# ingonyama-zk/blaze

Hardware: AMD Instinct MI355X
Metric: BLS12-381 MSM/s at 2^26 (higher is better)
Workload: dtype u32 registers holding 28-bit limbs (381-bit Fq, Montgomery)

## Files before the change

blaze_amd/_lib.py:

```python
from __future__ import annotations

import ctypes as C
import os

_HERE = os.path.dirname(os.path.abspath(__file__))
LIB_PATH = os.environ.get("BLAZE_HIP_LIB") or os.path.join(_HERE, "lib", "libblaze_hip.so")


class DriverClientError(Exception):

    VARIANTS = {
        1: "WriteError",
        2: "ReadError",
        3: "HBICAPNotReady",
        4: "InvalidPrimitiveParam",
        5: "CsvError",
        6: "LoadFailed",
        7: "FileError",
        8: "Unknown",
    }

    def __init__(self, code: int, message: str):
        self.code = code
        self.variant = self.VARIANTS.get(code, "Unknown")
# ... 99 lines not shown
    "blz_poseidon_wait_result": (C.c_int, [C.c_void_p]),
    "blz_poseidon_num_pending_results": (C.c_int, [C.c_void_p, C.POINTER(C.c_uint32)]),
    "blz_poseidon_raw_results": (C.c_int, [C.c_void_p, C.c_uint32, _u8p, C.c_size_t]),
    "blz_poseidon_result": (C.c_int, [C.c_void_p, C.c_uint32, _u8p, C.c_size_t, C.POINTER(C.c_uint32)]),
    "blz_poseidon_tree_device": (C.c_int, [C.c_void_p, C.c_void_p, C.c_size_t]),
    "blz_poseidon_counters": (C.c_int, [C.c_void_p, C.POINTER(C.c_uint32)]),
    "blz_poseidon_info": (C.c_int, [C.c_void_p, C.POINTER(C.c_uint64)]),
    "blz_poseidon_set_round_plan": (C.c_int, [C.c_void_p, C.c_int]),
    "blz_poseidon_prepare_round_plan": (C.c_int, [C.c_void_p, C.POINTER(C.c_uint32)]),
    "blz_poseidon_last_kernel_ms": (C.c_int, [C.c_void_p, C.POINTER(C.c_float)]),
    "blz_poseidon_stream": (C.c_int, [C.c_void_p, C.POINTER(C.c_void_p), C.POINTER(C.c_int)]),
    "blz_poseidon_reset": (C.c_int, [C.c_void_p]),
    "blz_device_malloc": (C.c_int, [C.c_int, C.c_size_t, C.POINTER(C.c_void_p)]),
    "blz_device_free": (C.c_int, [C.c_int, C.c_void_p]),
    "blz_host_malloc": (C.c_int, [C.c_int, C.c_size_t, C.POINTER(C.c_void_p)]),
    "blz_host_free": (C.c_int, [C.c_void_p]),
    "blz_memcpy_h2d": (C.c_int, [C.c_int, C.c_void_p, _u8p, C.c_size_t]),
    "blz_memcpy_d2h": (C.c_int, [C.c_int, _u8p, C.c_void_p, C.c_size_t]),
}
EXPORTED_SYMBOLS = tuple(_SIGS)
_AUX_SIGS = {
    "blz_synth_scalars": (C.c_int, [C.c_int, C.c_int, C.c_void_p, C.c_uint64, C.c_uint64]),
    "blz_synth_scalars_at": (C.c_int, [C.c_int, C.c_int, C.c_void_p, C.c_uint64, C.c_uint64, C.c_uint64]),
    "blz_synth_points": (C.c_int, [C.c_int, C.c_int, C.c_void_p, C.c_uint64, C.c_int, C.c_uint64]),
    "blz_synth_field_elements": (C.c_int, [C.c_int, C.c_void_p, C.c_uint64, C.c_uint64]),
    "blz_calib_mad_rate": (C.c_int, [C.c_int, C.c_uint32, C.POINTER(C.c_double)]),
    "blz_test_msm_stall": (C.c_int, [C.c_void_p, C.c_uint32, C.POINTER(C.c_void_p)]),
    "blz_test_ntt_stall": (C.c_int, [C.c_void_p, C.c_uint32, C.POINTER(C.c_void_p)]),
    "blz_test_stall_release": (C.c_int, [C.c_void_p]),
    "blz_test_field_op": (C.c_int, [C.c_int, C.c_int, C.c_int, C.c_int, _u8p, _u8p, _u8p, C.c_size_t]),
    "blz_test_ec_op": (C.c_int, [C.c_int, C.c_int, C.c_int, _u8p, _u8p, _u8p, _u8p, _u8p, C.c_size_t]),
    "blz_test_msm_tail_plan": (C.c_int, [C.c_int, C.c_int, C.c_uint32, C.c_int, C.c_int, C.c_int, C.c_int, C.c_int, C.POINTER(C.c_uint32), C.POINTER(C.c_uint8),
                                         C.c_char_p, C.c_size_t]),
    "blz_test_poseidon_permute": (C.c_int, [C.c_int, C.c_int, _u8p, C.c_size_t, C.c_int, _u8p, _u8p, C.c_size_t]),
    "blz_test_poseidon_hash": (C.c_int, [C.c_int, C.c_int, _u8p, C.c_size_t, C.c_int, _u8p, _u8p, C.c_size_t]),
    "blz_test_poseidon_hash_plan": (C.c_int, [C.c_int, C.c_int, _u8p, C.c_size_t, C.c_int, _u8p, _u8p, C.c_size_t, C.POINTER(C.c_uint32)]),
    "blz_test_poseidon_tree_check": (C.c_int, [C.c_int, C.c_int, _u8p, C.c_size_t, C.c_int, C.c_uint32, C.c_void_p, C.c_void_p, C.POINTER(C.c_uint64)]),
}
AUX_EXPORTED_SYMBOLS = tuple(_AUX_SIGS)


def lib():
    global _lib
    if _lib is None:
        if not os.path.exists(LIB_PATH):
            raise RuntimeError(
                f"{LIB_PATH} is missing: build it with `make -C blaze_amd/csrc` "
                "(or __graft_entry__.build()); blaze_amd has no CPU fallback"
            )
        L = C.CDLL(LIB_PATH, mode=C.RTLD_GLOBAL)
        for name, (res, args) in _SIGS.items():
            fn = getattr(L, name)
            fn.restype = res
            fn.argtypes = args
        _lib = L
    return _lib


def aux():
    global _aux
    if _aux is None:
        lib()
        path = LIB_PATH[:-3] + "_aux.so"
        if not os.path.exists(path):
            raise RuntimeError(f"{path} is missing: build it with `make -C blaze_amd/csrc`")
        A = C.CDLL(path)
# ... 93 lines not shown
```

blaze_amd/csrc/msm.hip:

```cpp
#include "msm_engine.hpp"
#include <mutex>
#include "field.hip.hpp"
#include "msm_digits.hip.hpp"

namespace blz {

size_t fq_bytes(int curve) { return curve == BLZ_BN254 ? 32 : 48; }
size_t mont_point_bytes(int curve) { return curve == BLZ_BN254 ? 64 : 128; }

static MsmPlan search_plan(uint32_t npts, int sbits, int ebits, int force_c, int split_ns, int max_w) {
    MsmPlan best;
    double best_cost = 1e300;
    const double t_entry = 0.163, t_bucket = 0.62, t_empty = 0.03, t_hot = 0.01;
    const int need = sbits + 1;
    const double t_split = (double)split_ns;
    for (int cmin = 3; cmin <= 23; ++cmin) {
        if (force_c > 0 && cmin != force_c) continue;
        for (int W = 1; W <= max_w; ++W) {
            if ((uint64_t)npts * W > MSM_MAX_ENTRIES) break;
            const int lower = W - 1;
            for (int k = 0; k <= lower; ++k) {
                if (force_c > 0 && k != 0) break;
                if (k > 0 && cmin + 1 > 23) break;
                const int low_bits = lower * cmin + k;
// ... 592 lines not shown
}

int MsmEngine::sync_all() {
    BLZ_TRY(use_device(device));
    BLZ_TRY(sync_stream_bounded(stream, "reset: main stream"));
    BLZ_TRY(sync_stream_bounded(tail_stream, "reset: tail stream"));
    BLZ_TRY(sync_stream_bounded(aux_stream, "reset: exchange stream"));
    BLZ_TRY(sync_stream_bounded(sort_stream, "reset: sort stream"));
    for (auto& S : slots) { S.busy = false; S.open = false; S.task_inputs_event = nullptr; }
    return BLZ_OK;
}

int MsmEngine::points_to_mont(const void* d_raw, void* d_mont, uint32_t npts) {
    BLZ_TRY(use_device(device));
    return msm_ops_for(curve, repr)->points_to_mont(*this, d_raw, d_mont, npts);
}

int MsmEngine::points_to_mont_even(const void* d_raw, void* d_mont, uint32_t nq) {
    BLZ_TRY(use_device(device));
    return msm_ops_for(curve, repr)->points_to_mont_even(*this, d_raw, d_mont, nq);
}
int MsmEngine::check_precompute(const void* d_raw, uint64_t nelem, uint32_t* flag, hipStream_t st) {
    BLZ_TRY(use_device(device));
    return msm_ops_for(curve, 0)->check_precompute(*this, d_raw, nelem, flag, st);
}

int MsmEngine::build_table(const void* d_raw, void* d_table, uint32_t npts, int c, int W, int base_shift, void* scratch, uint32_t* flag,
                           hipStream_t st) {
    BLZ_TRY(use_device(device));
    return msm_ops_for(curve, repr)->build_table(*this, d_raw, d_table, npts, c, W, base_shift, scratch, flag, st);
}
size_t MsmEngine::table_scratch_bytes(int W) const { return msm_ops_for(curve, repr)->table_scratch_bytes(W); }

static bool sort_fits_beside(int av, int sv) {
    const int a = (av + 7) & ~7, s = (sv + 7) & ~7;
    int waves = 512 / a;
    if (waves > 4) waves = 4;
    if (waves < 1) waves = 1;
    return waves * a + s <= 512 - 32;
}

static const int kScalarFieldBits[3] = {253, 255, 254};

MsmPlan MsmEngine::plan_for(uint32_t npts, int sbits) const {
    const int ebits = sbits == 256 ? kScalarFieldBits[curve] : sbits;
    return make_plan(npts, sbits, ebits, plan_override("c", 0));
}

static MsmPlan range_plan(int curve, uint32_t npts, int bit_lo, int bit_hi) {
    const int vbits = bit_hi - bit_lo;
    int ebits = kScalarFieldBits[curve] - bit_lo;
    if (ebits > vbits) ebits = vbits;
    if (ebits < 1) ebits = 1;
    MsmPlan P = make_plan(npts, vbits, ebits, plan_override("c", 0));
    P.base_bit = bit_lo;
    return P;
}
MsmPlan MsmEngine::plan_for_range(uint32_t npts, int bit_lo, int bit_hi) const { return range_plan(curve, npts, bit_lo, bit_hi); }

int msm_task_plan(int curve, uint32_t npts, int sbits, int table_c, int bit_lo, int bit_hi, MsmPlan& P, bool* ranged_out) {
    if (curve < 0 || curve > 2) return fail(BLZ_ERR_INVALID_PARAM, "unknown curve %d", curve);
    const int ebits = sbits == 256 ? kScalarFieldBits[curve] : sbits;
    const bool ranged = bit_hi > bit_lo && !(bit_lo == 0 && bit_hi >= sbits);
    if (ranged && (sbits != 256 || (bit_lo & 31) || (bit_hi & 31) || bit_hi > 256))
        return fail(BLZ_ERR_INVALID_PARAM, "scalar range [%d, %d): 32-bit aligned ranges of 256-bit scalars", bit_lo, bit_hi);
    P = table_c > 0 ? make_table_plan(npts, table_c, ranged ? bit_hi - bit_lo + 1 : 257)
        : ranged    ? range_plan(curve, npts, bit_lo, bit_hi)
                    : make_plan(npts, sbits, ebits, plan_override("c", 0));
    if (P.c == 0) return fail(BLZ_ERR_INVALID_PARAM, "no window plan for npts=%u sbits=%d%s", npts, sbits, table_c > 0 ? " (window table)" : "");
    if (P.table && !msm_sort3_ok(P, sbits)) return fail(BLZ_ERR_INVALID_PARAM, "window-table task outside the sort's range (c=%d)", P.c);
    P.L = (uint32_t)plan_override("L", (int)P.L);
    if (P.L < 1) P.L = 1;
// ... 9 lines not shown
    const uint32_t per = (uint32_t)(((2ull * P.npts + halves - 1) / halves + 15) & ~(uint64_t)15);
    if (want > 1) want = (int)(((uint64_t)P.npts + per - 1) / per);
    *per_out = want > 1 ? per : P.npts;
    return want;
}

int MsmEngine::begin(uint32_t npts, int sbits, int* slot_out, int table_c, int bit_lo, int bit_hi, int nslices, bool phased) {
    BLZ_TRY(use_device(device));
    const MsmCurveOps* ops = msm_ops_for(curve, repr);
    hipStream_t st = stream;
    if (npts == 0) return fail(BLZ_ERR_INVALID_PARAM, "begin: empty task");
    int slot = (cur + 1) % MSM_QUEUE_DEPTH;
    if (slots[slot].busy) slot = (slot + 1) % MSM_QUEUE_DEPTH;
    if (slots[slot].busy) return fail(BLZ_ERR_INVALID_PARAM, "task queue full (%d tasks in flight)", MSM_QUEUE_DEPTH);
    MsmSlot& S = slots[slot];
    MsmPlan P;
    bool ranged = false;
    BLZ_TRY(msm_task_plan(curve, npts, sbits, table_c, bit_lo, bit_hi, P, &ranged));
    const uint64_t G = P.G;
    uint32_t per = npts;
    nslices = msm_task_pieces(P, nslices, phased, &per);
    BLZ_TRY(plan_tail(P, ops->tail, nslices > 1, S.tail));
    BLZ_LOG(2, "msm plan: npts=%u sbits=%d c=%d W=%d Bw=%u G=%llu L=%u pieces=%d tail: %s", npts, sbits, P.c, P.W, P.Bw,
            (unsigned long long)G, P.L, nslices, describe(S.tail).c_str());
    const uint64_t max_entries = (uint64_t)per * P.W;
    const uint64_t max_units = G + max_entries / P.L + 1;
    if (max_units >= (1ull << 32)) return fail(BLZ_ERR_INVALID_PARAM, "unit bound %llu exceeds 32 bits", (unsigned long long)max_units);

    const int hide_env = env_int("BLAZE_SORT_HIDE", 1);
    const MsmSlot& O = slots[(slot + 1) % MSM_QUEUE_DEPTH];
    bool s3 = P.table || (hide_env != 0 && nslices == 1 && msm_sort3_ok(P, sbits));
    bool fits = true;
    auto sort_fits = [&](bool table) {
        const int av = ops->accumulate_vgprs(), sv = msm_sort3_max_vgprs(table);
        return !(av > 0 && sv > 0 && !sort_fits_beside(av, sv));
    };
    if (s3 && hide_env == 1 && !P.table) {
        if (recent_hot[0] || recent_hot[1]) s3 = false;
    }
    if (s3 && hide_env == 1) {
        fits = sort_fits(P.table);
        if (!fits && !P.table) s3 = false;
    }
    bool hide = s3 && O.busy && hide_env != 0 && fits;
    const bool pingpong = nslices > 1 && hide_env != 0 && !O.busy && !P.table && msm_sort3_ok(P, sbits) && !(recent_hot[0] || recent_hot[1]) &&
                          sort_fits(false);
    if (pingpong) { s3 = true; hide = true; }

    cur = slot;
    if (slot_out) *slot_out = slot;
    last_plan = S.plan = P;
    S.npts = npts;
    S.sbits = sbits;
    S.ranged = ranged;
    S.bit_lo = bit_lo;
    S.bit_hi = bit_hi;
    S.repr = repr;
    S.slices = nslices;
    S.pts_per_slice = per;
    S.max_units = max_units;
    S.use_s3 = s3 && (hide || hide_env == 2 || P.table);
    S.sort_hidden = hide;
    S.pingpong = pingpong;
    S.acc_pp_recorded[0] = S.acc_pp_recorded[1] = false;
    S.phased = phased;
    S.task_inputs_event = inputs_event;
    S.accum_timed = false;
    BLZ_HIP(hipEventRecord(S.ev[0], st), BLZ_ERR_UNKNOWN);
// ... 230 lines not shown
```

blaze_amd/csrc/msm_engine.hpp:

```cpp
#pragma once
#include "common.hpp"

namespace blz {

constexpr int MSM_MAX_W = 96;
constexpr uint64_t MSM_MAX_ENTRIES = (1ull << 32) - (1ull << 26);
struct MsmPlan {
    uint32_t npts = 0;
    int sbits = 256;
    int c = 0;
    int W = 0;
    uint8_t width[MSM_MAX_W] = {};
    uint32_t boff[MSM_MAX_W + 1] = {};
    uint32_t Bw = 0;
    int Wv = 0;
    uint64_t G = 0;
    uint32_t L = 0;
    bool table = false;
    int ebits = 0;
    int base_bit = 0;
    double cost = 0;
};
MsmPlan make_plan(uint32_t npts, int sbits, int ebits, int force_c);
int table_window_bits(uint32_t npts, int need_bits = 257);
// ... 94 lines not shown
    bool last_sort_hidden = false;
    bool recent_hot[2] = {false, false};
    uint32_t sort_slices = 1, sort_nc = 0;
    int sort_cl = 0;
    void* sort_inter_fine = nullptr;

    int init(int device_id, int curve_id, int precompute_factor);
    bool destroy();
    uint32_t* slot_result(int s) { return result.as<uint32_t>() + (size_t)s * 64; }
    bool can_accept() const;
    MsmPlan plan_for(uint32_t npts, int sbits) const;
    int points_to_mont(const void* d_raw, void* d_mont, uint32_t npts);
    int points_to_mont_even(const void* d_raw, void* d_mont, uint32_t nq);
    int check_precompute(const void* d_raw, uint64_t nelem, uint32_t* flag, hipStream_t st);
    int build_table(const void* d_raw, void* d_table, uint32_t npts, int c, int W, int base_shift, void* scratch, uint32_t* flag,
                    hipStream_t st);
    size_t table_scratch_bytes(int W) const;
    int run(const void* d_points_mont, const void* d_scalars, uint32_t npts, int sbits, int* slot, int table_c = 0, int bit_lo = 0,
            int bit_hi = 0);
    MsmPlan plan_for_range(uint32_t npts, int bit_lo, int bit_hi) const;
    int finish(int slot, uint8_t* out);
    int combine_partials(const uint8_t* partials, size_t count, uint8_t* out, bool on_device);
    int sync_all();
};

int msm_points_from_mont(int format_id, const void* d_mont, void* d_raw, uint64_t npts, hipStream_t st);
int msm_points_all_canonical(int format_id, const void* d_raw, uint64_t npts, uint32_t* flag, hipStream_t st);
int copy_words_to_pinned(void* host_pinned, const void* d_src, uint32_t dwords, hipStream_t st);
size_t fq_bytes(int curve);
size_t mont_point_bytes(int curve);
int msm_sort_lds(MsmEngine& E, const void* d_scalars, uint32_t npts, int sbits);
bool msm_sort3_ok(const MsmPlan& P, int sbits);
int msm_sort3_max_vgprs(bool table);
int msm_sort3(MsmEngine& E, const void* d_scalars, uint32_t npts, int sbits);
int msm_sort_lds_scatter(MsmEngine& E);
bool msm_sort_tiny_ok(const MsmPlan& P, uint32_t npts, int sbits);
int msm_sort_tiny(MsmEngine& E, const void* d_scalars, uint32_t npts, int sbits, uint32_t max_units);
int launch_fill_units(MsmEngine& E, uint32_t units);

struct MsmCurveOps {
    int (*points_to_mont)(MsmEngine&, const void* d_raw, void* d_mont, uint32_t npts);
    int (*emit_infinity)(MsmEngine&);
    int (*run_accumulate)(MsmEngine&, MsmSlot&, const void* d_pts, uint32_t max_units, int slice);
    int (*merge_buckets)(MsmEngine&);
    int (*run_reduce)(MsmEngine&, MsmSlot&, const void* sums, const void* unit_off);
    TailTraits tail;
    int (*accumulate_vgprs)();
    int (*build_table)(MsmEngine&, const void* d_raw, void* d_table, uint32_t npts, int c, int W, int base_shift, void* scratch,
                       uint32_t* flag, hipStream_t st);
    size_t (*table_scratch_bytes)(int W);
    int (*combine)(MsmEngine&, const uint8_t* partials, size_t count, uint8_t* out, bool on_device);
    int (*points_to_mont_even)(MsmEngine&, const void* d_raw, void* d_mont, uint32_t nq);
    int (*check_precompute)(MsmEngine&, const void* d_raw, uint64_t nelem, uint32_t* flag, hipStream_t st);
    int (*points_from_mont)(const void* d_mont, void* d_raw, uint64_t npts, hipStream_t st);
    int (*points_all_canonical)(const void* d_raw, uint64_t npts, uint32_t* flag, hipStream_t st);
};
const MsmCurveOps& msm_ops_bls377();
const MsmCurveOps& msm_ops_bls381();
const MsmCurveOps& msm_ops_bn254();
const MsmCurveOps& msm_ops_bn254_w32();
const MsmCurveOps* msm_ops_for(int curve, int repr = 0);

}
```

blaze_amd/csrc/msm_impl.hip.hpp:

```cpp
#pragma once
#include "msm_engine.hpp"
#include "ec.hip.hpp"
#include "ec_rr.hip.hpp"
#include "ec_quad.hip.hpp"
#include "ec_row.hip.hpp"
#include <type_traits>

namespace blz {

template <class F>
constexpr int MONT_STRIDE = 2 * F::N > 16 ? 32 : 2 * F::N;

template <class F>
constexpr bool rr_point_packed() {
    if constexpr (USE_RR<F>) return 2 * F::RR::NL > MONT_STRIDE<F>;
    else return false;
}

template <class F>
BLZ_DEV void store_mont_point(uint32_t* __restrict__ mont, size_t p, Fp<F>& x, Fp<F>& y) {
    if constexpr (USE_RR<F>) {
        using Q = typename F::RR;
        Frr<Q, 1, 2> xr, yr;
        rr_to_mont_from_words<Q>(xr, x.v);
// ... 299 lines not shown
    if constexpr (USE_RR<F>) {
        XYZZRR<typename F::RR> r;
        ptrr_from_xyzz32<F>(r, a);
        ptrr_store(partial, idx, r);
    } else {
        uint32_t* q = partial + idx * 4 * F::N;
        fp_store(q, a.x); fp_store(q + F::N, a.y); fp_store(q + 2 * F::N, a.zz); fp_store(q + 3 * F::N, a.zzz);
    }
}

template <class F>
BLZ_DEV void load_affine(Affine<F>& a, const uint32_t* pts, uint32_t idx) {
    const uint32_t* q = pts + (size_t)idx * MONT_STRIDE<F>;
    fp_load(a.x, q);
    fp_load(a.y, q + F::N);
}
template <class F>
BLZ_DEV void load_xyzz(XYZZ<F>& a, const uint32_t* base, size_t idx) {
    const uint32_t* q = base + idx * 4 * F::N;
    fp_load(a.x, q);
    fp_load(a.y, q + F::N);
    fp_load(a.zz, q + 2 * F::N);
    fp_load(a.zzz, q + 3 * F::N);
}
template <class F>
BLZ_DEV void store_xyzz(uint32_t* base, size_t idx, const XYZZ<F>& a) {
    uint32_t* q = base + idx * 4 * F::N;
    fp_store(q, a.x);
    fp_store(q + F::N, a.y);
    fp_store(q + 2 * F::N, a.zz);
    fp_store(q + 3 * F::N, a.zzz);
}

#ifndef BLZ_ACC_RR_WAVES
#define BLZ_ACC_RR_WAVES 2
#endif
#ifndef BLZ_ACC_W32_WAVES
#define BLZ_ACC_W32_WAVES 2
#endif
#ifndef BLZ_ACC_VGPR_CAP
#define BLZ_ACC_VGPR_CAP 100
#endif
#ifdef BLZ_GATHER_MASK
#define BLZ_PT_IDX(e) ((e) & 0x7fffffffu & (uint32_t)(BLZ_GATHER_MASK))
#else
#define BLZ_PT_IDX(e) ((e) & 0x7fffffffu)
#endif
template <class F, bool CONT>
BLZ_DEV void accumulate_body(const uint32_t* __restrict__ pts, const uint32_t* __restrict__ entries,
                             const uint32_t* __restrict__ off, const uint32_t* __restrict__ unit_off,
                             const uint32_t* __restrict__ unit_bucket, const uint32_t* __restrict__ unit_order,
                             const uint32_t* __restrict__ stats, uint32_t L, uint32_t* __restrict__ partial,
                             uint32_t* __restrict__ sums, bool first) {
    uint32_t t = blockIdx.x * 128u + threadIdx.x;
    if (t >= stats[0]) return;
    const uint32_t u = unit_order[t];
    uint32_t g = unit_bucket[u];
    const uint32_t u0 = unit_off[g];
    uint32_t k = u - u0;
    uint32_t start = off[g] + k * L;
    uint32_t end = off[g + 1];
    if (end - start > L) end = start + L;
    uint32_t* dst = partial;
    size_t didx = u;
    bool resume = false;
    if constexpr (CONT) {
        if (unit_off[g + 1] - u0 == 1) {
            dst = sums;
            didx = g;
            resume = !first;
        }
    }
    if constexpr (USE_RR<F>) {
        using Q = typename F::RR;
        XYZZRR<Q> acc;
        ptrr_set_inf(acc);
        if constexpr (CONT) {
            if (resume) ptrr_load(acc, sums, g);
        }
        uint32_t e = entries[start];
#if BLZ_ACC_RR_WAVES == 2
        uint32_t en = start + 1 < end ? entries[start + 1] : 0u;
        AffineRR<Q> nxt;
        load_affine_rr<F>(nxt, pts, BLZ_PT_IDX(e));
        uint32_t j = start;
#ifndef BLZ_ACC_NO_AADD
        if ((!CONT || first) && end - start >= 2) {
            const AffineRR<Q> p0 = nxt;
            const bool neg0 = (e & 0x80000000u) != 0;
            const uint32_t e1 = en;
            AffineRR<Q> p1;
            load_affine_rr<F>(p1, pts, BLZ_PT_IDX(e1));
            if (start + 2 < end) {
                e = entries[start + 2];
                load_affine_rr<F>(nxt, pts, BLZ_PT_IDX(e));
                en = start + 3 < end ? entries[start + 3] : 0u;
            }
            ptrr_aadd<Q, 1>(acc, p0, neg0, p1, (e1 & 0x80000000u) != 0);
            j = start + 2;
        }
#endif
        for (; j < end; ++j) {
            const AffineRR<Q> cur = nxt;
            const bool neg = (e & 0x80000000u) != 0;
            if (j + 1 < end) {
                e = en;
                load_affine_rr<F>(nxt, pts, BLZ_PT_IDX(e));
                if (j + 2 < end) en = entries[j + 2];
            }
            ptrr_madd<Q, 1>(acc, cur, neg);
        }
// ... 892 lines not shown
    hipLaunchKernelGGL(k_points_all_canonical<F>, dim3((unsigned)((npts + 255) / 256)), dim3(256), 0, st, (const uint32_t*)d_raw, npts, flag);
    BLZ_HIP(hipGetLastError(), BLZ_ERR_UNKNOWN);
    return BLZ_OK;
}

constexpr uint32_t CHECK_BLOCKS = 256 * 4 * 3;
template <class F>
int points_to_mont_even_t(MsmEngine& E, const void* d_raw, void* d_mont, uint32_t nq) {
    if (nq == 0) return BLZ_OK;
    hipLaunchKernelGGL(k_points_to_mont_even<F>, dim3((nq + 255) / 256), dim3(256), 0, E.stream, (const uint32_t*)d_raw, (uint32_t*)d_mont, nq);
    BLZ_HIP(hipGetLastError(), BLZ_ERR_UNKNOWN);
    return BLZ_OK;
}
template <class F>
int check_precompute_t(MsmEngine& E, const void* d_raw, uint64_t nelem, uint32_t* flag, hipStream_t st) {
    (void)E;
    if (nelem == 0) return BLZ_OK;
    const uint64_t want = (nelem * 7u + 63u) / 64u;
    const uint32_t blocks = (uint32_t)(want < CHECK_BLOCKS ? want : CHECK_BLOCKS);
    hipLaunchKernelGGL(k_check_precompute<F>, dim3(blocks), dim3(64), 0, st, (const uint32_t*)d_raw, nelem, flag);
    BLZ_HIP(hipGetLastError(), BLZ_ERR_UNKNOWN);
    return BLZ_OK;
}

template <class F>
int accumulate_vgprs_t() {
    hipFuncAttributes a;
    if (hipFuncGetAttributes(&a, (const void*)k_accumulate<F>) != hipSuccess) {
        (void)hipGetLastError();
        return 0;
    }
    return a.numRegs;
}

template <class F>
MsmCurveOps make_ops() {
    MsmCurveOps o;
    o.points_to_mont = &points_to_mont_t<F>;
    o.emit_infinity = &emit_infinity_t<F>;
    o.run_accumulate = &run_accumulate_t<F>;
    o.merge_buckets = &merge_buckets_t<F>;
    o.run_reduce = &run_reduce_t<F>;
    o.tail = TailTraits{HAS_RR<F>, HAS_ROW<F>, partial_dwords<F>()};
    o.accumulate_vgprs = &accumulate_vgprs_t<F>;
    o.build_table = &build_table_t<F>;
    o.table_scratch_bytes = &table_scratch_bytes_t<F>;
    o.combine = &combine_t<F>;
    o.points_to_mont_even = &points_to_mont_even_t<F>;
    o.check_precompute = &check_precompute_t<F>;
    o.points_from_mont = &points_from_mont_t<F>;
    o.points_all_canonical = &points_all_canonical_t<F>;
    return o;
}

}
```

blaze_amd/csrc/msm_sort3.hip:

```cpp
#include "msm_engine.hpp"
#include "msm_digits.hip.hpp"

namespace blz {

constexpr int S3_THREADS = 256;
constexpr int S3_SH1 = 14;
constexpr int S3_SH2 = 7;
constexpr int S3_T = 12;
constexpr int S3_PB = S3_THREADS * S3_T;
constexpr uint32_t S3_SLICE2 = 4096;
constexpr int S3_T2 = S3_SLICE2 / S3_THREADS;
constexpr int S3_T3 = 28;
constexpr uint32_t S3_R3 = S3_THREADS * S3_T3;
constexpr uint32_t S3_MAXNB1 = 2048;
constexpr uint32_t S3_CNT_PTS = 16384;
constexpr uint32_t S3T_IMG = 12288;

struct S3Geom {
    int W, prio;
    uint32_t NB1;
    uint8_t width[MSM_MAX_W];
    uint16_t bitoff[MSM_MAX_W];
    uint16_t binoff1[MSM_MAX_W + 1];
    static constexpr bool TABLE = false;
    static constexpr uint32_t HIST1 = S3_MAXNB1;
    using Win = int;
    __device__ int cw(int w) const { return width[w]; }
    __device__ uint32_t first_bin(int w) const { return binoff1[w]; }
    __device__ static constexpr uint32_t shift1() { return S3_SH1; }
    static constexpr uint32_t bits3() { return S3_SH2; }
    __device__ static uint32_t index1(uint32_t p, uint32_t, uint32_t) { return p; }
    __device__ static uint32_t rem1(uint32_t rem) { return rem; }
    struct L2 {
        int prio;
        using Lo = uint8_t;
        static constexpr uint32_t TAB2 = 128;
        static constexpr uint32_t KY_D = 8, KY_R = 16;
        static constexpr uint32_t LO_MASK = 127u;
        __device__ static constexpr uint32_t shift2() { return S3_SH2; }
        __device__ static constexpr uint32_t bits2() { return S3_SH1 - S3_SH2; }
        __device__ static uint32_t low2(uint32_t r, uint32_t) { return r & 127u; }
// ... 567 lines not shown
    S3TGeom g;
    g.W = P.W;
    g.c = P.c;
    g.prio = exp_knob("BLAZE_SORT_PRIO", 3);
    g.sh1 = (uint32_t)(P.c - 1 - 8);
    g.NB1 = (uint32_t)(P.G >> g.sh1);
    const double per_bucket = (double)npts * P.W / (double)P.G;
    int b3 = 4;
    while (b3 < 10 && (double)(2u << b3) * per_bucket <= 6144.0) ++b3;
    if ((uint32_t)b3 > g.sh1) b3 = (int)g.sh1;
    int b2 = (int)g.sh1 - b3;
    if (b2 > 8) { b2 = 8; b3 = (int)g.sh1 - 8; }
    g.b2 = (uint32_t)b2;
    g.b3 = (uint32_t)b3;
    g.xs = g.sh1 > 16 ? g.sh1 - 16 : 0;
    return g;
}

bool msm_sort3_ok(const MsmPlan& P, int sbits) {
    if (P.table) {
        if (sbits != 256 || P.sbits < 1 || P.sbits > 256 || P.c < 16 || P.c > 26 || P.W * P.c < P.sbits + 1) return false;
        if ((uint64_t)P.npts * P.W >= (1ull << 30)) return false;
        const S3TGeom g = s3t_geometry(P, P.npts);
        return g.NB1 <= 256 && g.b2 <= 8 && g.b3 >= 1 && g.b3 <= 10 && g.xs <= 1 && g.b3 > g.xs;
    }
    if ((sbits != 256 && sbits != 64 && sbits != 32) || P.W < 1) return false;
    for (int w = 0; w < P.W; ++w)
        if (P.width[w] < S3_SH1 + 1 || P.width[w] > 23) return false;
    if ((P.G >> S3_SH1) > S3_MAXNB1 || (P.G & ((1u << S3_SH1) - 1u))) return false;
    if ((P.G >> S3_SH2) > 2048u * 256u) return false;
    return true;
}

int msm_sort3_max_vgprs(bool table) {
    using L2 = S3Geom::L2;
    static const void* const plain_ks[] = {(const void*)k3_l1_count<S3Geom, 8>, (const void*)k3_l1_scatter<S3Geom, 8>,
                                           (const void*)k3_l1_count<S3Geom, 1>, (const void*)k3_l1_scatter<S3Geom, 1>,
                                           (const void*)k3_l1_count<S3Geom, 2>, (const void*)k3_l1_scatter<S3Geom, 2>,
                                           (const void*)k3_l2_count<L2>, (const void*)k3_l2_scatter<L2>, (const void*)k3_l3};
    static const void* const table_ks[] = {(const void*)k3_l1_count<S3TGeom, 8>, (const void*)k3_l1_scatter<S3TGeom, 8>,
                                           (const void*)k3_l2_count<S3TGeom>, (const void*)k3_l2_scatter<S3TGeom>,
                                           (const void*)k3t_l3<true>, (const void*)k3t_l3<false>};
    static int cached[2] = {-1, -1};
    int& c = cached[table ? 1 : 0];
    if (c >= 0) return c;
    const void* const* ks = table ? table_ks : plain_ks;
    const size_t n = table ? sizeof(table_ks) / sizeof(*table_ks) : sizeof(plain_ks) / sizeof(*plain_ks);
    int mx = 0;
    for (size_t i = 0; i < n; ++i) {
        hipFuncAttributes a;
        if (hipFuncGetAttributes(&a, ks[i]) != hipSuccess) {
            (void)hipGetLastError();
            return c = 0;
        }
        if (a.numRegs > mx) mx = a.numRegs;
    }
    return c = mx;
}

template <class Geom, int NW>
static int s3_level1(hipStream_t st, const uint32_t* sc, uint32_t npts, const Geom& g, uint32_t* cnt1, uint32_t* off1, uint32_t* cur1,
                     uint32_t* i1_idx, uint16_t* i1_rem) {
    const dim3 blk(S3_THREADS);
    const size_t lds1 = (size_t)((NW + 2) * S3_PB + 3 * 256) * 4;
    hipLaunchKernelGGL((k3_l1_count<Geom, NW>), dim3((npts + S3_CNT_PTS - 1) / S3_CNT_PTS), blk, 0, st, sc, npts, g, cnt1);
    hipLaunchKernelGGL(k3_scan_small, dim3(1), blk, 0, st, cnt1, g.NB1, off1, cur1, g.prio);
    BLZ_TRY(ensure_dynamic_lds((const void*)k3_l1_scatter<Geom, NW>, (int)lds1));
    hipLaunchKernelGGL((k3_l1_scatter<Geom, NW>), dim3((npts + S3_PB - 1) / S3_PB), blk, lds1, st, sc, npts, g, cur1, i1_idx, i1_rem);
    return BLZ_OK;
}

template <class Geom>
static int s3_enqueue(MsmEngine& E, const Geom& g, const void* d_scalars, uint32_t npts, int sbits) {
    using L2 = typename Geom::L2;
    using Lo = typename L2::Lo;
    const MsmPlan& P = E.last_plan;
    hipStream_t st = E.sort_st;
    MsmEngine::SortBufs& B = E.sb();
    const uint32_t NB1 = g.NB1, NB2 = (uint32_t)(P.G >> g.bits3());
    const uint64_t max_entries = (uint64_t)npts * P.W;
    const uint32_t max_items = (uint32_t)(max_entries / S3_SLICE2) + NB1 + 1;
    const uint32_t nsb = (NB2 + 2047u) / 2048u;
    if (Geom::TABLE && nsb > 256) return fail(BLZ_ERR_UNKNOWN, "window-table sort: %u final-level bins exceed the scan's range", NB2);
    const size_t tab_dw = (size_t)3 * (NB1 + 2) + (size_t)3 * (NB2 + 2) + 260 + 4 + 2 * ((size_t)max_items + 2);
    BLZ_TRY(E.sort3_tabs.reserve(tab_dw * 4));
    uint32_t* cnt1 = E.sort3_tabs.as<uint32_t>();
    uint32_t* off1 = cnt1 + NB1 + 2;
    uint32_t* cur1 = off1 + NB1 + 2;
    uint32_t* cnt2 = cur1 + NB1 + 2;
    uint32_t* off2 = cnt2 + NB2 + 2;
    uint32_t* cur2 = off2 + NB2 + 2;
    uint32_t* bsum = cur2 + NB2 + 2;
    uint32_t* nitems = bsum + 260;
    uint2* map = reinterpret_cast<uint2*>(nitems + 4);
    BLZ_TRY(E.inter.reserve(max_entries * 6 + 64));
    BLZ_TRY(E.inter2.reserve(max_entries * (4 + sizeof(Lo)) + 64));
    uint32_t* i1_idx = E.inter.as<uint32_t>();
// ... 43 lines not shown
```

blaze_amd/csrc/testhooks.hip:

```cpp
#include "common.hpp"
#include "ec_rr.hip.hpp"
#include "ec_row.hip.hpp"
#include "poseidon_engine.hpp"
#include "msm_engine.hpp"

namespace blz {

template <class P>
__global__ __launch_bounds__(64) void k_test_field(int op, const uint32_t* a, const uint32_t* b, uint32_t* out, uint32_t n) {
    uint32_t i = blockIdx.x * 64u + threadIdx.x;
    if (i >= n) return;
    Fp<P> x, y, r;
    fp_load(x, a + (size_t)i * P::N);
    fp_load(y, b + (size_t)i * P::N);
    fp_to_mont(x, x);
    fp_to_mont(y, y);
    switch (op) {
        case 0: fp_mul(r, x, y); break;
        case 1: fp_add(r, x, y); break;
        case 2: fp_sub(r, x, y); break;
        case 3: fp_inv(r, x); break;
        case 5:
        case 6:
            if constexpr (P::LAZY) {
// ... 553 lines not shown
                                 const void* d_records, uint64_t out[2]) {
    if (!words || !d_input || !d_records || !out) return fail(BLZ_ERR_INVALID_PARAM, "null argument");
    if (tree_height < 1 || tree_height > 11) return fail(BLZ_ERR_INVALID_PARAM, "tree height out of range");
    BLZ_TRY(blz_poseidon_check_words(field, tree_mode, words, len, nullptr));
    BLZ_TRY(use_device(device_id));
    switch (field) {
        case BLZ_BLS377: return test_pos_tree_check_t<Fr_BLS377>(words, len, tree_mode, tree_height, d_input, d_records, out);
        case BLZ_BLS381: return test_pos_tree_check_t<Fr_BLS381>(words, len, tree_mode, tree_height, d_input, d_records, out);
        case BLZ_BN254: return test_pos_tree_check_t<Fr_BN254>(words, len, tree_mode, tree_height, d_input, d_records, out);
    }
    return fail(BLZ_ERR_INVALID_PARAM, "unknown field %d", field);
}

int blz_test_msm_tail_plan(int curve, int repr, uint32_t npts, int sbits, int pieces, int table_c, int bit_lo, int bit_hi, uint32_t plan_out[8],
                           uint8_t* widths, char* text, size_t cap) {
    if (!plan_out || !text || cap == 0) return fail(BLZ_ERR_INVALID_PARAM, "null argument");
    const MsmCurveOps* ops = msm_ops_for(curve, repr);
    if (!ops || npts == 0) return fail(BLZ_ERR_INVALID_PARAM, "unknown curve %d or empty task", curve);
    MsmPlan P;
    BLZ_TRY(msm_task_plan(curve, npts, sbits, table_c, bit_lo, bit_hi, P, nullptr));
    uint32_t per = 0;
    pieces = msm_task_pieces(P, pieces, false, &per);
    TailPlan T;
    BLZ_TRY(plan_tail(P, ops->tail, pieces > 1, T));
    const uint32_t out[8] = {(uint32_t)P.c, (uint32_t)P.W, (uint32_t)P.G, P.L, P.Bw, (uint32_t)P.Wv, (uint32_t)P.ebits, P.table ? 1u : 0u};
    memcpy(plan_out, out, sizeof(out));
    if (widths) memcpy(widths, P.width, (size_t)P.W);
    const std::string line = describe(T);
    if (line.size() >= cap) return fail(BLZ_ERR_INVALID_PARAM, "text buffer of %zu bytes for a line of %zu", cap, line.size());
    memcpy(text, line.c_str(), line.size() + 1);
    return BLZ_OK;
}

}
```

include/blaze_hip_aux.h:

```cpp
#ifndef BLAZE_HIP_AUX_H
#define BLAZE_HIP_AUX_H

#include "blaze_hip.h"

#ifdef __cplusplus
extern "C" {
#endif


int blz_synth_scalars(int device_id, int curve, void* d_out, uint64_t n, uint64_t seed);
int blz_synth_scalars_at(int device_id, int curve, void* d_out, uint64_t n, uint64_t seed, uint64_t start);
int blz_synth_points(int device_id, int curve, void* d_out, uint64_t n, int pf, uint64_t start);
int blz_synth_field_elements(int device_id, void* d_out, uint64_t n, uint64_t seed);

int blz_calib_mad_rate(int device_id, uint32_t target_ms, double out[4]);

int blz_test_msm_stall(blz_msm* h, uint32_t max_ms, void** token);
int blz_test_ntt_stall(blz_ntt* h, uint32_t max_ms, void** token);
int blz_test_stall_release(void* token);

int blz_test_field_op(int device_id, int curve, int field, int op, const uint8_t* a, const uint8_t* b,
                      uint8_t* out, size_t n);
int blz_test_ec_op(int device_id, int curve, int op, const uint8_t* p, const uint8_t* q,
                   const uint8_t* inf_flags, uint8_t* out, uint8_t* out_inf, size_t n);

int blz_test_msm_tail_plan(int curve, int repr, uint32_t npts, int sbits, int pieces, int table_c, int bit_lo, int bit_hi, uint32_t plan_out[8],
                           uint8_t* widths, char* text, size_t cap);

int blz_test_poseidon_permute(int device_id, int field, const uint8_t* words, size_t len, int t, const uint8_t* states_in,
                              uint8_t* states_out, size_t n);
int blz_test_poseidon_hash(int device_id, int field, const uint8_t* words, size_t len, int t, const uint8_t* inputs, uint8_t* digests,
                           size_t n);
int blz_test_poseidon_hash_plan(int device_id, int field, const uint8_t* words, size_t len, int t, const uint8_t* inputs, uint8_t* digests,
                                size_t n, uint32_t* state);
int blz_test_poseidon_tree_check(int device_id, int field, const uint8_t* words, size_t len, int tree_mode, uint32_t tree_height,
                                 const void* d_input, const void* d_records, uint64_t out[2]);

#ifdef __cplusplus
}
#endif
#endif
```

Before: 8.520.

## Gather bucket-accumulate points into LDS via async global_load_lds lines

In the RR accumulate kernel, each wave now brings point rows into LDS with global_load_lds. Lanes cooperatively fetch 128-byte point lines, using ds_swizzle to broadcast addresses, and the next point's load is double-buffered ahead of the madd. This is meant to replace scattered per-lane global point loads with coalesced line loads overlapped with arithmetic. The sort-hiding fit check now also counts LDS usage of the accumulate and sort3 kernels, and the sort3 per-thread tile drops from 12 to 8 so it fits beside the new LDS image. The costs are more LDS pressure, wave-uniform loop control where shorter buckets idle, and a hand-encoded gfx9 waitcnt.

Result: faster. 8.643 (median of 6 runs) (+1.4%).

```diff
diff --git a/blaze_amd/_lib.py b/blaze_amd/_lib.py
--- a/blaze_amd/_lib.py
+++ b/blaze_amd/_lib.py
@@ -155,6 +155,7 @@
     "blz_test_ec_op": (C.c_int, [C.c_int, C.c_int, C.c_int, _u8p, _u8p, _u8p, _u8p, _u8p, C.c_size_t]),
     "blz_test_msm_tail_plan": (C.c_int, [C.c_int, C.c_int, C.c_uint32, C.c_int, C.c_int, C.c_int, C.c_int, C.c_int, C.POINTER(C.c_uint32), C.POINTER(C.c_uint8),
                                          C.c_char_p, C.c_size_t]),
+    "blz_test_sort_fits_beside": (C.c_int, [C.c_int, C.c_int, C.c_int, C.c_int]),
     "blz_test_poseidon_permute": (C.c_int, [C.c_int, C.c_int, _u8p, C.c_size_t, C.c_int, _u8p, _u8p, C.c_size_t]),
     "blz_test_poseidon_hash": (C.c_int, [C.c_int, C.c_int, _u8p, C.c_size_t, C.c_int, _u8p, _u8p, C.c_size_t]),
     "blz_test_poseidon_hash_plan": (C.c_int, [C.c_int, C.c_int, _u8p, C.c_size_t, C.c_int, _u8p, _u8p, C.c_size_t, C.POINTER(C.c_uint32)]),
diff --git a/blaze_amd/csrc/msm.hip b/blaze_amd/csrc/msm.hip
--- a/blaze_amd/csrc/msm.hip
+++ b/blaze_amd/csrc/msm.hip
@@ -648,12 +648,16 @@
 }
 size_t MsmEngine::table_scratch_bytes(int W) const { return msm_ops_for(curve, repr)->table_scratch_bytes(W); }
 
-static bool sort_fits_beside(int av, int sv) {
+bool msm_sort_fits_beside(int av, int sv, int al, int sl) {
+    if (av <= 0 || sv <= 0) return true;
     const int a = (av + 7) & ~7, s = (sv + 7) & ~7;
     int waves = 512 / a;
     if (waves > 4) waves = 4;
     if (waves < 1) waves = 1;
-    return waves * a + s <= 512 - 32;
+    if (waves * a + s > 512 - 32) return false;
+    if (al <= 0 || sl <= 0) return true;
+    const int ak = (al + 1023) >> 10, sk = (sl + 1023) >> 10;
+    return 2 * waves * ak + sk <= 160;
 }
 
 static const int kScalarFieldBits[3] = {253, 255, 254};
@@ -729,8 +733,7 @@
     bool s3 = P.table || (hide_env != 0 && nslices == 1 && msm_sort3_ok(P, sbits));
     bool fits = true;
     auto sort_fits = [&](bool table) {
-        const int av = ops->accumulate_vgprs(), sv = msm_sort3_max_vgprs(table);
-        return !(av > 0 && sv > 0 && !sort_fits_beside(av, sv));
+        return msm_sort_fits_beside(ops->accumulate_vgprs(), msm_sort3_max_vgprs(table), ops->accumulate_lds(), msm_sort3_max_lds(table));
     };
     if (s3 && hide_env == 1 && !P.table) {
         if (recent_hot[0] || recent_hot[1]) s3 = false;
diff --git a/blaze_amd/csrc/msm_engine.hpp b/blaze_amd/csrc/msm_engine.hpp
--- a/blaze_amd/csrc/msm_engine.hpp
+++ b/blaze_amd/csrc/msm_engine.hpp
@@ -150,6 +150,8 @@
 int msm_sort_lds(MsmEngine& E, const void* d_scalars, uint32_t npts, int sbits);
 bool msm_sort3_ok(const MsmPlan& P, int sbits);
 int msm_sort3_max_vgprs(bool table);
+int msm_sort3_max_lds(bool table);
+bool msm_sort_fits_beside(int av, int sv, int al, int sl);
 int msm_sort3(MsmEngine& E, const void* d_scalars, uint32_t npts, int sbits);
 int msm_sort_lds_scatter(MsmEngine& E);
 bool msm_sort_tiny_ok(const MsmPlan& P, uint32_t npts, int sbits);
@@ -164,6 +166,7 @@
     int (*run_reduce)(MsmEngine&, MsmSlot&, const void* sums, const void* unit_off);
     TailTraits tail;
     int (*accumulate_vgprs)();
+    int (*accumulate_lds)();
     int (*build_table)(MsmEngine&, const void* d_raw, void* d_table, uint32_t npts, int c, int W, int base_shift, void* scratch,
                        uint32_t* flag, hipStream_t st);
     size_t (*table_scratch_bytes)(int W);
diff --git a/blaze_amd/csrc/msm_impl.hip.hpp b/blaze_amd/csrc/msm_impl.hip.hpp
--- a/blaze_amd/csrc/msm_impl.hip.hpp
+++ b/blaze_amd/csrc/msm_impl.hip.hpp
@@ -355,6 +355,52 @@
     fp_store(q + 3 * F::N, a.zzz);
 }
 
+template <class F>
+constexpr bool acc_gather_lines() {
+    if constexpr (USE_RR<F>) return !rr_point_packed<F>() && MONT_STRIDE<F> == 32 && F::RR::NL == 14;
+    else return false;
+}
+constexpr int ACC_IMG_PIECES = 512;
+template <int K>
+BLZ_DEV void acc_lines_issue_one(uint32_t lds, uint32_t lo, uint32_t hi, uint32_t piece) {
+    constexpr int pattern = (K << 5) | 0x18;
+    const uint32_t olo = (uint32_t)__builtin_amdgcn_ds_swizzle((int)lo, pattern);
+    const uint32_t ohi = (uint32_t)__builtin_amdgcn_ds_swizzle((int)hi, pattern);
+    const uint64_t src = (((uint64_t)ohi << 32) | olo) + piece;
+    __builtin_amdgcn_global_load_lds((const __attribute__((address_space(1))) void*)src,
+                                     (__attribute__((address_space(3))) void*)(uintptr_t)(lds + K * 1024), 16, 0, 0);
+}
+BLZ_DEV void acc_lines_issue(uint32_t lds, const uint32_t* pts, uint32_t idx) {
+    const uint64_t line = (uint64_t)(uintptr_t)pts + (uint64_t)idx * 128u;
+    const uint32_t lo = (uint32_t)line, hi = (uint32_t)(line >> 32), piece = (threadIdx.x & 7u) * 16u;
+    acc_lines_issue_one<0>(lds, lo, hi, piece); acc_lines_issue_one<1>(lds, lo, hi, piece);
+    acc_lines_issue_one<2>(lds, lo, hi, piece); acc_lines_issue_one<3>(lds, lo, hi, piece);
+    acc_lines_issue_one<4>(lds, lo, hi, piece); acc_lines_issue_one<5>(lds, lo, hi, piece);
+    acc_lines_issue_one<6>(lds, lo, hi, piece); acc_lines_issue_one<7>(lds, lo, hi, piece);
+}
+BLZ_DEV uint32_t acc_image_base(const uint4* img) {
+    return (uint32_t)__builtin_amdgcn_readfirstlane((int)(uint32_t)(uintptr_t)(const __attribute__((address_space(3))) void*)img);
+}
+template <class Q>
+BLZ_DEV void acc_lines_read(AffineRR<Q>& a, const uint4* img) {
+    const uint32_t lane = threadIdx.x & 63u;
+    const uint4* q4 = img + (lane & 7u) * 64 + (lane >> 3) * 8;
+    uint32_t w[2 * Q::NL];
+#if defined(__HIP_DEVICE_COMPILE__) && !defined(__GFX9__)
+#error "acc_lines_read: the s_waitcnt immediate is written in the gfx9 encoding"
+#endif
+    __builtin_amdgcn_s_waitcnt(0x0F70);
+    asm volatile("" ::: "memory");
+#pragma unroll
+    for (int i = 0; i < 2 * Q::NL / 4; ++i) {
+        uint4 v = q4[i];
+        w[4 * i] = v.x; w[4 * i + 1] = v.y; w[4 * i + 2] = v.z; w[4 * i + 3] = v.w;
+    }
+    asm volatile("s_waitcnt lgkmcnt(0)" ::: "memory");
+#pragma unroll
+    for (int i = 0; i < Q::NL; ++i) { a.x.v[i] = w[i]; a.y.v[i] = w[Q::NL + i]; }
+}
+
 #ifndef BLZ_ACC_RR_WAVES
 #define BLZ_ACC_RR_WAVES 2
 #endif
@@ -376,22 +422,33 @@
                              const uint32_t* __restrict__ stats, uint32_t L, uint32_t* __restrict__ partial,
                              uint32_t* __restrict__ sums, bool first) {
     uint32_t t = blockIdx.x * 128u + threadIdx.x;
-    if (t >= stats[0]) return;
-    const uint32_t u = unit_order[t];
-    uint32_t g = unit_bucket[u];
-    const uint32_t u0 = unit_off[g];
-    uint32_t k = u - u0;
-    uint32_t start = off[g] + k * L;
-    uint32_t end = off[g + 1];
-    if (end - start > L) end = start + L;
+#if BLZ_ACC_RR_WAVES == 2
+    constexpr bool LINES = acc_gather_lines<F>();
+#else
+    constexpr bool LINES = false;
+#endif
+    const uint32_t nunits = stats[0];
+    if ((LINES ? t & ~63u : t) >= nunits) return;
+    const bool live = t < nunits;
+    uint32_t g = 0, start = 0, end = 0;
     uint32_t* dst = partial;
-    size_t didx = u;
+    size_t didx = 0;
     bool resume = false;
-    if constexpr (CONT) {
-        if (unit_off[g + 1] - u0 == 1) {
-            dst = sums;
-            didx = g;
-            resume = !first;
+    if (live) {
+        const uint32_t u = unit_order[t];
+        g = unit_bucket[u];
+        const uint32_t u0 = unit_off[g];
+        const uint32_t k = u - u0;
+        start = off[g] + k * L;
+        end = off[g + 1];
+        if (end - start > L) end = start + L;
+        didx = u;
+        if constexpr (CONT) {
+            if (unit_off[g + 1] - u0 == 1) {
+                dst = sums;
+                didx = g;
+                resume = !first;
+            }
         }
     }
     if constexpr (USE_RR<F>) {
@@ -400,6 +457,50 @@
         ptrr_set_inf(acc);
         if constexpr (CONT) {
             if (resume) ptrr_load(acc, sums, g);
+        }
+        if constexpr (LINES) {
+            __shared__ uint4 images[2 * ACC_IMG_PIECES];
+            const uint4* img = images + (threadIdx.x >> 6) * ACC_IMG_PIECES;
+            const uint32_t lds = acc_image_base(img);
+            uint32_t j = start;
+            uint32_t e = j < end ? entries[j] : 0u;
+            uint32_t en = j + 1 < end ? entries[j + 1] : 0u;
+            acc_lines_issue(lds, pts, BLZ_PT_IDX(e));
+            if (live && start == end) ptrr_store(dst, didx, acc);
+#ifndef BLZ_ACC_NO_AADD
+            const bool aadd = (!CONT || first) && end - start >= 2;
+            if (__any(aadd)) {
+                AffineRR<Q> p0, p1;
+                acc_lines_read(p0, img);
+                const bool neg0 = (e & 0x80000000u) != 0;
+                const uint32_t e1 = aadd ? en : e;
+                acc_lines_issue(lds, pts, BLZ_PT_IDX(e1));
+                if (aadd) {
+                    j = start + 2;
+                    e = j < end ? entries[j] : 0u;
+                    en = j + 1 < end ? entries[j + 1] : 0u;
+                }
+                acc_lines_read(p1, img);
+                if (__any(j < end)) acc_lines_issue(lds, pts, BLZ_PT_IDX(e));
+                if (aadd) {
+                    ptrr_aadd<Q, 1>(acc, p0, neg0, p1, (e1 & 0x80000000u) != 0);
+                    if (j == end) ptrr_store(dst, didx, acc);
+                }
+            }
+#endif
+            while (__any(j < end)) {
+                AffineRR<Q> cur;
+                acc_lines_read(cur, img);
+                const bool neg = (e & 0x80000000u) != 0;
+                const bool more = j + 1 < end;
+                e = more ? en : 0u;
+                if (__any(more)) acc_lines_issue(lds, pts, BLZ_PT_IDX(e));
+                if (j + 2 < end) en = entries[j + 2];
+                ptrr_madd<Q, 1>(acc, cur, neg);
+                ++j;
+                if (j == end) ptrr_store(dst, didx, acc);
+            }
+            return;
         }
         uint32_t e = entries[start];
 #if BLZ_ACC_RR_WAVES == 2
@@ -1358,6 +1459,15 @@
     }
     return a.numRegs;
 }
+template <class F>
+int accumulate_lds_t() {
+    hipFuncAttributes a;
+    if (hipFuncGetAttributes(&a, (const void*)k_accumulate<F>) != hipSuccess) {
+        (void)hipGetLastError();
+        return -1;
+    }
+    return (int)a.sharedSizeBytes;
+}
 
 template <class F>
 MsmCurveOps make_ops() {
@@ -1369,6 +1479,7 @@
     o.run_reduce = &run_reduce_t<F>;
     o.tail = TailTraits{HAS_RR<F>, HAS_ROW<F>, partial_dwords<F>()};
     o.accumulate_vgprs = &accumulate_vgprs_t<F>;
+    o.accumulate_lds = &accumulate_lds_t<F>;
     o.build_table = &build_table_t<F>;
     o.table_scratch_bytes = &table_scratch_bytes_t<F>;
     o.combine = &combine_t<F>;
diff --git a/blaze_amd/csrc/msm_sort3.hip b/blaze_amd/csrc/msm_sort3.hip
--- a/blaze_amd/csrc/msm_sort3.hip
+++ b/blaze_amd/csrc/msm_sort3.hip
@@ -6,7 +6,10 @@
 constexpr int S3_THREADS = 256;
 constexpr int S3_SH1 = 14;
 constexpr int S3_SH2 = 7;
-constexpr int S3_T = 12;
+#ifndef BLZ_S3_T
+#define BLZ_S3_T 8
+#endif
+constexpr int S3_T = BLZ_S3_T;
 constexpr int S3_PB = S3_THREADS * S3_T;
 constexpr uint32_t S3_SLICE2 = 4096;
 constexpr int S3_T2 = S3_SLICE2 / S3_THREADS;
@@ -640,37 +643,44 @@
     return true;
 }
 
-int msm_sort3_max_vgprs(bool table) {
+static constexpr size_t s3_lds1(int nw) { return (size_t)((nw + 2) * S3_PB + 3 * 256) * 4; }
+struct S3Need { int vgprs, lds; };
+static S3Need s3_needs(bool table) {
     using L2 = S3Geom::L2;
-    static const void* const plain_ks[] = {(const void*)k3_l1_count<S3Geom, 8>, (const void*)k3_l1_scatter<S3Geom, 8>,
-                                           (const void*)k3_l1_count<S3Geom, 1>, (const void*)k3_l1_scatter<S3Geom, 1>,
-                                           (const void*)k3_l1_count<S3Geom, 2>, (const void*)k3_l1_scatter<S3Geom, 2>,
-                                           (const void*)k3_l2_count<L2>, (const void*)k3_l2_scatter<L2>, (const void*)k3_l3};
-    static const void* const table_ks[] = {(const void*)k3_l1_count<S3TGeom, 8>, (const void*)k3_l1_scatter<S3TGeom, 8>,
-                                           (const void*)k3_l2_count<S3TGeom>, (const void*)k3_l2_scatter<S3TGeom>,
-                                           (const void*)k3t_l3<true>, (const void*)k3t_l3<false>};
-    static int cached[2] = {-1, -1};
-    int& c = cached[table ? 1 : 0];
-    if (c >= 0) return c;
-    const void* const* ks = table ? table_ks : plain_ks;
+    struct K { const void* f; size_t dyn; };
+    static const K plain_ks[] = {{(const void*)k3_l1_count<S3Geom, 8>, 0}, {(const void*)k3_l1_scatter<S3Geom, 8>, s3_lds1(8)},
+                                 {(const void*)k3_l1_count<S3Geom, 1>, 0}, {(const void*)k3_l1_scatter<S3Geom, 1>, s3_lds1(1)},
+                                 {(const void*)k3_l1_count<S3Geom, 2>, 0}, {(const void*)k3_l1_scatter<S3Geom, 2>, s3_lds1(2)},
+                                 {(const void*)k3_l2_count<L2>, 0}, {(const void*)k3_l2_scatter<L2>, 0}, {(const void*)k3_l3, 0}};
+    static const K table_ks[] = {{(const void*)k3_l1_count<S3TGeom, 8>, 0}, {(const void*)k3_l1_scatter<S3TGeom, 8>, s3_lds1(8)},
+                                 {(const void*)k3_l2_count<S3TGeom>, 0}, {(const void*)k3_l2_scatter<S3TGeom>, 0},
+                                 {(const void*)k3t_l3<true>, (size_t)S3_R3 * 4}, {(const void*)k3t_l3<false>, (size_t)S3T_IMG * 4}};
+    static S3Need cached[2] = {{-1, -1}, {-1, -1}};
+    S3Need& c = cached[table ? 1 : 0];
+    if (c.vgprs >= 0) return c;
+    const K* ks = table ? table_ks : plain_ks;
     const size_t n = table ? sizeof(table_ks) / sizeof(*table_ks) : sizeof(plain_ks) / sizeof(*plain_ks);
-    int mx = 0;
+    S3Need mx = {0, 0};
     for (size_t i = 0; i < n; ++i) {
         hipFuncAttributes a;
-        if (hipFuncGetAttributes(&a, ks[i]) != hipSuccess) {
+        if (hipFuncGetAttributes(&a, ks[i].f) != hipSuccess) {
             (void)hipGetLastError();
-            return c = 0;
-        }
-        if (a.numRegs > mx) mx = a.numRegs;
+            return c = S3Need{0, 0};
+        }
+        if (a.numRegs > mx.vgprs) mx.vgprs = a.numRegs;
+        const int lds = (int)(a.sharedSizeBytes + ks[i].dyn);
+        if (lds > mx.lds) mx.lds = lds;
     }
     return c = mx;
 }
+int msm_sort3_max_vgprs(bool table) { return s3_needs(table).vgprs; }
+int msm_sort3_max_lds(bool table) { return s3_needs(table).lds; }
 
 template <class Geom, int NW>
 static int s3_level1(hipStream_t st, const uint32_t* sc, uint32_t npts, const Geom& g, uint32_t* cnt1, uint32_t* off1, uint32_t* cur1,
                      uint32_t* i1_idx, uint16_t* i1_rem) {
     const dim3 blk(S3_THREADS);
-    const size_t lds1 = (size_t)((NW + 2) * S3_PB + 3 * 256) * 4;
+    const size_t lds1 = s3_lds1(NW);
     hipLaunchKernelGGL((k3_l1_count<Geom, NW>), dim3((npts + S3_CNT_PTS - 1) / S3_CNT_PTS), blk, 0, st, sc, npts, g, cnt1);
     hipLaunchKernelGGL(k3_scan_small, dim3(1), blk, 0, st, cnt1, g.NB1, off1, cur1, g.prio);
     BLZ_TRY(ensure_dynamic_lds((const void*)k3_l1_scatter<Geom, NW>, (int)lds1));
diff --git a/blaze_amd/csrc/testhooks.hip b/blaze_amd/csrc/testhooks.hip
--- a/blaze_amd/csrc/testhooks.hip
+++ b/blaze_amd/csrc/testhooks.hip
@@ -609,4 +609,8 @@
     return BLZ_OK;
 }
 
-}
+int blz_test_sort_fits_beside(int acc_vgprs, int sort_vgprs, int acc_lds, int sort_lds) {
+    return msm_sort_fits_beside(acc_vgprs, sort_vgprs, acc_lds, sort_lds) ? 1 : 0;
+}
+
+}
diff --git a/include/blaze_hip_aux.h b/include/blaze_hip_aux.h
--- a/include/blaze_hip_aux.h
+++ b/include/blaze_hip_aux.h
@@ -27,6 +27,8 @@
 int blz_test_msm_tail_plan(int curve, int repr, uint32_t npts, int sbits, int pieces, int table_c, int bit_lo, int bit_hi, uint32_t plan_out[8],
                            uint8_t* widths, char* text, size_t cap);
 
+int blz_test_sort_fits_beside(int acc_vgprs, int sort_vgprs, int acc_lds, int sort_lds);
+
 int blz_test_poseidon_permute(int device_id, int field, const uint8_t* words, size_t len, int t, const uint8_t* states_in,
                               uint8_t* states_out, size_t n);
 int blz_test_poseidon_hash(int device_id, int field, const uint8_t* words, size_t len, int t, const uint8_t* inputs, uint8_t* digests,
```
